# lpylpy0514/VitTracker

Hardware: AMD Instinct MI355X
Metric: track() frames/sec per GPU, vit_48_h32, 128px search / 64px template (higher is better)
Workload: dtype f32

## Files before the change

### vittracker_amd/csrc/vt_head3.h

```cpp
#pragma once
#include "vt_bf3.h"
#include "vt_head.h"

#ifndef VT_F16
#ifndef VT_SEQ3_C2_MAXP
#define VT_SEQ3_C2_MAXP 5
#endif
#ifndef VT_SEQ3_C2_ACT
#define VT_SEQ3_C2_ACT 8
#endif
#ifndef VT_H3_SKIP
#define VT_H3_SKIP 0
#endif
namespace vth3 {

using vth::C;
using vth::W1;
using vth::nchunks;
using vth::ntiles;
using vt3::bf16x8;
using vt3::u32x2;
using vt3::u32x4;
using vt3::split3;
using vt3::join3;
using G = vth::Geo<8>;

constexpr int npairs(int cin) { return (nchunks(cin) + 1) / 2; }
constexpr int img16(int cin, int cout) { return ntiles(cout) * npairs(cin) * 3 * 64; }
constexpr int O3_W1 = 0;
constexpr int O3_W2 = O3_W1 + img16(48, 32);
constexpr int O3_W3 = O3_W2 + img16(32, 16);
constexpr int O3_W4 = O3_W3 + img16(16, 8);
constexpr int TOWER3_STRIDE = O3_W4 + img16(8, 4);

template <int CIN, int COUT, int NW = 4, int ACT = NW, int MAXP_ = 2>
struct HeadConv3 {
    static constexpr int NQ = CIN / 4, NQO = COUT / 4, NCH = nchunks(CIN), NCP = npairs(CIN), NOT = ntiles(COUT);
    static constexpr bool SPLIT_OT = NOT == 2;
    static constexpr int TSTEP = SPLIT_OT ? NW / 2 : ACT;
    static constexpr int NPT = G::NT / TSTEP;
    static_assert(G::NT % TSTEP == 0 && NPT >= 1 && NOT <= 2, "work split");
    static constexpr int MAXP = NCP < MAXP_ ? NCP : MAXP_;
    static constexpr int NPASS = (NCP + MAXP - 1) / MAXP;
    static constexpr int PS_IN = NQ * G::NPIX, PS_OUT = NQO * G::NPIX;
    u32x4 a[2][MAXP][3];

    __device__ __forceinline__ const u32x4* wbase(const u32x4* __restrict__ wimg, int wave) const {
        return wimg + (SPLIT_OT ? (size_t)(wave & 1) * NCP * 192 : 0);
    }
    __device__ __forceinline__ void load_pass(const u32x4* __restrict__ wb, int p0, int n, int lane, u32x4 (&dst)[MAXP][3]) {
#pragma unroll
        for (int k = 0; k < MAXP; ++k)
            if (k < n)
#pragma unroll
                for (int pc = 0; pc < 3; ++pc) dst[k][pc] = wb[((size_t)(p0 + k) * 3 + pc) * 64 + lane];
        __builtin_amdgcn_sched_barrier(0);
    }
    __device__ __forceinline__ void prefetch(const u32x4* __restrict__ wimg, int wave, int lane) {
        load_pass(wbase(wimg, wave), 0, MAXP, lane, a[0]);
    }
    template <bool FIRST = false>
    __device__ __forceinline__ void run(const u32x2* in_map, u32x2* out_map, const u32x4* __restrict__ wimg,
                                        const float* __restrict__ bias, int wave, int lane) {
        if (!SPLIT_OT && wave >= ACT) return;
        if constexpr (FIRST) prefetch(wimg, wave, lane);
        const int q = lane >> 4;
        const int ot = SPLIT_OT ? (wave & 1) : 0, tfirst = SPLIT_OT ? (wave >> 1) : wave;
        f4 acc[NPT];
        const f4 bv = ld4(bias + 16 * ot + 4 * q);
#pragma unroll
        for (int i = 0; i < NPT; ++i) acc[i] = bv;
        const u32x4* __restrict__ wb = wbase(wimg, wave);
        int cb[NPT][3], centre[NPT];
#pragma unroll
        for (int i = 0; i < NPT; ++i) { G::tap_cols(tfirst + TSTEP * i, lane, cb[i]); centre[i] = cb[i][1] + G::P; }
        auto at = [&](int c, int i) {
            int tap, icq;
            if constexpr (NQ % 4 == 0) { const int cc = c < NCH ? c : NCH - 1; tap = (4 * cc) / NQ; icq = 4 * cc - tap * NQ + q; }
            else vtc::decode_quad<NQ>(4 * c + q, tap, icq);
            const int dy = tap / 3, dx = tap - 3 * dy;
            return icq * G::NPIX + dy * G::P + (dx == 0 ? cb[i][0] : (dx == 1 ? cb[i][1] : cb[i][2]));
        };
        auto read_b = [&](int cp, u32x4 (&b)[NPT][3]) {
#pragma unroll
            for (int i = 0; i < NPT; ++i) {
                const int o0 = at(2 * cp, i), o1 = at(2 * cp + 1, i);
#pragma unroll
                for (int pc = 0; pc < 3; ++pc) {
                    const u32x2 lo = in_map[pc * PS_IN + o0], hi = in_map[pc * PS_IN + o1];
                    b[i][pc] = u32x4{lo.x, lo.y, hi.x, hi.y};
                }
            }
        };
        u32x4 b[2][NPT][3];
        read_b(0, b[0]);
#pragma unroll
        for (int p = 0; p < NPASS; ++p) {
            constexpr int LASTN = NCP - (NPASS - 1) * MAXP;
            const int n = p + 1 < NPASS ? MAXP : LASTN;
            if (p + 1 < NPASS) load_pass(wb, (p + 1) * MAXP, p + 2 < NPASS ? MAXP : LASTN, lane, a[(p + 1) & 1]);
#pragma unroll
            for (int k = 0; k < MAXP; ++k) {
                if (k >= n) break;
                const int cp = p * MAXP + k;
                if (cp + 1 < NCP) {
                    read_b(cp + 1, b[(cp + 1) & 1]);
                    __builtin_amdgcn_sched_barrier(0);
                }
                const u32x4 (&w)[3] = a[p & 1][k];
#pragma unroll
                for (int i = 0; i < NPT; ++i) {
                    const u32x4 (&x)[3] = b[cp & 1][i];
                    auto mm = [&](int wp, int xp) {
                        acc[i] = __builtin_amdgcn_mfma_f32_16x16x32_bf16(__builtin_bit_cast(bf16x8, w[wp]), __builtin_bit_cast(bf16x8, x[xp]), acc[i], 0, 0, 0);
                    };
                    mm(2, 0); mm(0, 2); mm(1, 1); mm(1, 0); mm(0, 1); mm(0, 0);
                }
            }
        }
        if (16 * ot + 4 * q < COUT) {
#pragma unroll
            for (int i = 0; i < NPT; ++i) {
                f4 v = acc[i];
                v.x = fmaxf(v.x, 0.f); v.y = fmaxf(v.y, 0.f); v.z = fmaxf(v.z, 0.f); v.w = fmaxf(v.w, 0.f);
                u32x2 h, m, l;
                split3(v, h, m, l);
                const int e = (4 * ot + q) * G::NPIX + centre[i];
                out_map[e] = h; out_map[PS_OUT + e] = m; out_map[2 * PS_OUT + e] = l;
            }
        }
    }
    static constexpr int SP = 3, NSP = (NCP + SP - 1) / SP, SBUF16 = SP * 192;
    static constexpr int pass_n16(int p) { return (p + 1 < NSP ? SP : NCP - (NSP - 1) * SP) * 192; }
    template <typename Pipe>
    __device__ __forceinline__ void run_staged(const u32x2* in_map, u32x2* out_map, const float* __restrict__ bias, int wave, int lane,
                                               int g0, Pipe& pipe) {
        static_assert(NOT == 1 && NPT == 1 && ACT == NW, "staged form: one output tile, one pixel tile per wave");
        const int q = lane >> 4;
        f4 acc = ld4(bias + 4 * q);
        int cb[3];
        G::tap_cols(wave, lane, cb);
        const int centre = cb[1] + G::P;
        auto at = [&](int c) {
            int tap, icq;
            if constexpr (NQ % 4 == 0) { const int cc = c < NCH ? c : NCH - 1; tap = (4 * cc) / NQ; icq = 4 * cc - tap * NQ + q; }
            else vtc::decode_quad<NQ>(4 * c + q, tap, icq);
            const int dy = tap / 3, dx = tap - 3 * dy;
            return icq * G::NPIX + dy * G::P + (dx == 0 ? cb[0] : (dx == 1 ? cb[1] : cb[2]));
        };
        auto read_b = [&](int cp, u32x4 (&b)[3]) {
            const int o0 = at(2 * cp), o1 = at(2 * cp + 1);
#pragma unroll
            for (int pc = 0; pc < 3; ++pc) {
                const u32x2 lo = in_map[pc * PS_IN + o0], hi = in_map[pc * PS_IN + o1];
                b[pc] = u32x4{lo.x, lo.y, hi.x, hi.y};
            }
        };
        u32x4 b[2][3], w[2][3];
        read_b(0, b[0]);
#pragma unroll
        for (int p = 0; p < NSP; ++p) {
            const int n = pass_n16(p) / 192, g = g0 + p;
            pipe.fetch(g + 2);
            const u32x4* sb = pipe.buf(g);
            auto read_w = [&](int k, u32x4 (&ww)[3]) {
#pragma unroll
                for (int pc = 0; pc < 3; ++pc) ww[pc] = sb[(k * 3 + pc) * 64 + lane];
            };
            read_w(0, w[0]);
#pragma unroll
            for (int k = 0; k < SP; ++k) {
                if (k >= n) break;
                const int cp = p * SP + k;
                if (k + 1 < n) read_w(k + 1, w[(k + 1) & 1]);
                if (cp + 1 < NCP) read_b(cp + 1, b[(cp + 1) & 1]);
                __builtin_amdgcn_sched_barrier(0);
                const u32x4 (&x)[3] = b[cp & 1];
                const u32x4 (&ww)[3] = w[k & 1];
                auto mm = [&](int wp, int xp) {
                    acc = __builtin_amdgcn_mfma_f32_16x16x32_bf16(__builtin_bit_cast(bf16x8, ww[wp]), __builtin_bit_cast(bf16x8, x[xp]), acc, 0, 0, 0);
                };
                if (!(VT_H3_SKIP & 2)) { mm(2, 0); mm(0, 2); mm(1, 1); mm(1, 0); mm(0, 1); mm(0, 0); }
            }
            if (p == NSP - 1 && 4 * q < COUT) {
                f4 v = acc;
                v.x = fmaxf(v.x, 0.f); v.y = fmaxf(v.y, 0.f); v.z = fmaxf(v.z, 0.f); v.w = fmaxf(v.w, 0.f);
                u32x2 h, m, l;
                split3(v, h, m, l);
                const int e = q * G::NPIX + centre;
                out_map[e] = h; out_map[PS_OUT + e] = m; out_map[2 * PS_OUT + e] = l;
            }
            pipe.park(g + 1);
            __syncthreads();
        }
    }
};

constexpr int IN_E = 3 * (C / 4) * G::NPIX, M1_E = 3 * (W1 / 4) * G::NPIX, M2_E = 3 * 4 * G::NPIX;
constexpr int TOWERS3_LDS_BYTES = (IN_E + M1_E + M2_E) * 8;
constexpr int SBUF_BYTES = 3 * 192 * 16;
static_assert(IN_E * 8 / 3 >= SBUF_BYTES, "a tower's second staging buffer is its third of the input map (dead after conv1)");
constexpr int FUSED3_LDS_BYTES = (IN_E + 3 * (M1_E + M2_E)) * 8 + 5 * 64 * 4 + 3 * SBUF_BYTES;
static_assert(FUSED3_LDS_BYTES <= 160 * 1024, "LDS");

struct WeightPipe {
    static constexpr int N2 = HeadConv3<W1, 16>::NSP, N3 = HeadConv3<16, 8>::NSP, N4 = HeadConv3<8, 4>::NSP, NP = N2 + N3 + N4;
    const u32x4* tw3;
    u32x4 *buf0, *buf1;
    int tid;
    u32x4 r[2][3];
    static constexpr int off16(int j) {
        return j < N2 ? O3_W2 + j * HeadConv3<W1, 16>::SBUF16 : j < N2 + N3 ? O3_W3 + (j - N2) * HeadConv3<16, 8>::SBUF16 : O3_W4 + (j - N2 - N3) * HeadConv3<8, 4>::SBUF16;
    }
    static constexpr int n16(int j) {
        return j < N2 ? HeadConv3<W1, 16>::pass_n16(j) : j < N2 + N3 ? HeadConv3<16, 8>::pass_n16(j - N2) : HeadConv3<8, 4>::pass_n16(j - N2 - N3);
    }
    __device__ __forceinline__ const u32x4* buf(int j) const { return (j & 1) ? buf1 : buf0; }
    __device__ __forceinline__ void fetch(int j) {
        if (j >= NP) return;
        const u32x4* __restrict__ src = tw3 + off16(j);
#pragma unroll
        for (int k = 0; k < 3; ++k)
            if (tid + 256 * k < n16(j)) r[j & 1][k] = src[tid + 256 * k];
        __builtin_amdgcn_sched_barrier(0);
    }
    __device__ __forceinline__ void park(int j) {
        if (j >= NP) return;
        u32x4* dst = (j & 1) ? buf1 : buf0;
#pragma unroll
        for (int k = 0; k < 3; ++k)
            if (tid + 256 * k < n16(j)) dst[tid + 256 * k] = r[j & 1][k];
    }
};

__device__ __forceinline__ void stage_tokens(u32x2* in_map, const float* __restrict__ feat, int b, int item) {
    const int icq = item >> 6, pix = item & 63;
    u32x2 h, m, l;
    split3(ld4(feat + ((size_t)b * 64 + pix) * C + 4 * icq), h, m, l);
    const int e = icq * G::NPIX + G::interior(pix >> 3, pix & 7);
    in_map[e] = h; in_map[(C / 4) * G::NPIX + e] = m; in_map[2 * (C / 4) * G::NPIX + e] = l;
}

__global__ __launch_bounds__(256) void head_towers3_kernel(const float* __restrict__ feat, const float* __restrict__ hw,
                                                          const u32x4* __restrict__ hw3, float* __restrict__ score,
                                                          float* __restrict__ size, float* __restrict__ offset) {
    extern __shared__ __attribute__((aligned(16))) float sm[];
    u32x2* in_map = reinterpret_cast<u32x2*>(sm);
    u32x2* m1 = in_map + IN_E;
    u32x2* m2 = m1 + M1_E;
    const int b = blockIdx.x, t = blockIdx.y;
    const int lane = threadIdx.x & 63;
    const int wave = __builtin_amdgcn_readfirstlane(threadIdx.x >> 6);
    const float* __restrict__ tw = hw + (size_t)t * vth::TOWER_STRIDE;
    const u32x4* __restrict__ tw3 = hw3 + (size_t)t * TOWER3_STRIDE;
    HeadConv3<C, W1> c1;
    HeadConv3<W1, 16> c2;
    HeadConv3<16, 8> c3;
    HeadConv3<8, 4> c4;
    c1.prefetch(tw3 + O3_W1, wave, lane);
    for (int i = threadIdx.x; i < (IN_E + M1_E + M2_E) / 2; i += 256) reinterpret_cast<u32x4*>(in_map)[i] = u32x4{0, 0, 0, 0};
    __syncthreads();
    for (int i = threadIdx.x; i < 64 * (C / 4); i += 256) stage_tokens(in_map, feat, b, i);
    __syncthreads();
    c2.prefetch(tw3 + O3_W2, wave, lane);
    c1.run(in_map, m1, tw3 + O3_W1, tw + vth::O_B1, wave, lane);
    c3.prefetch(tw3 + O3_W3, wave, lane);
    __syncthreads();
    c2.run(m1, m2, tw3 + O3_W2, tw + vth::O_B2, wave, lane);
    c4.prefetch(tw3 + O3_W4, wave, lane);
    __syncthreads();
    c3.run(m2, m1, tw3 + O3_W3, tw + vth::O_B3, wave, lane);
    __syncthreads();
    c4.run(m1, m2, tw3 + O3_W4, tw + vth::O_B4, wave, lane);
    __syncthreads();
    if (threadIdx.x < 64) {
        const int pix = threadIdx.x, e = G::interior(pix >> 3, pix & 7);
        const f4 v = join3(m2[e], m2[G::NPIX + e], m2[2 * G::NPIX + e]);
        const int nout = (t == 0) ? 1 : 2;
        for (int o = 0; o < nout; ++o) {
            const f4 w5 = ld4(tw + vth::O_W5 + 4 * o);
            float y = tw[vth::O_B5 + o];
            y = fmaf(v.x, w5.x, y); y = fmaf(v.y, w5.y, y); y = fmaf(v.z, w5.z, y); y = fmaf(v.w, w5.w, y);
            if (t == 0) score[(size_t)b * 64 + pix] = sigmoid_clamped(y);
            else if (t == 2) size[((size_t)b * 2 + o) * 64 + pix] = sigmoid_clamped(y);
            else offset[((size_t)b * 2 + o) * 64 + pix] = y;
        }
    }
}

__global__ __launch_bounds__(768) void head_fused3_kernel(const float* __restrict__ feat, const float* __restrict__ hw,
                                                          const u32x4* __restrict__ hw3, const float* __restrict__ window,
                                                          float* __restrict__ score, float* __restrict__ size,
                                                          float* __restrict__ offset, float* __restrict__ pred,
                                                          float* __restrict__ hann, float* __restrict__ conf, TrackTail tail,
                                                          int has_tail) {
    constexpr int F = 8;
    extern __shared__ __attribute__((aligned(16))) float sm[];
    u32x2* in_map = reinterpret_cast<u32x2*>(sm);
    const int b = blockIdx.x;
    const int lane = threadIdx.x & 63;
    const int wave = __builtin_amdgcn_readfirstlane(threadIdx.x >> 6);
    const int t = wave >> 2, wv = wave & 3, tid = threadIdx.x - 256 * t;
    u32x2* m1 = in_map + IN_E + t * (M1_E + M2_E);
    u32x2* m2 = m1 + M1_E;
    float* outs = reinterpret_cast<float*>(in_map + IN_E + 3 * (M1_E + M2_E));
    const float* __restrict__ tw = hw + (size_t)t * vth::TOWER_STRIDE;
    const u32x4* __restrict__ tw3 = hw3 + (size_t)t * TOWER3_STRIDE;
    HeadConv3<C, W1, 4, 4, 1> c1;
    HeadConv3<W1, 16> c2;
    HeadConv3<16, 8> c3;
    HeadConv3<8, 4> c4;
    c1.prefetch(tw3 + O3_W1, wv, lane);
    static_assert(64 * (C / 4) == 768, "one staged element per thread");
    const f4 fv = ld4(feat + ((size_t)b * 64 + (threadIdx.x & 63)) * C + 4 * (threadIdx.x >> 6));
    float win = 0.f;
    if (wave == 0 && window != nullptr) win = window[lane];
    {
        constexpr int NPL = (IN_E + 3 * (M1_E + M2_E)) / G::NPIX, ZU = (G::NPIX - F * G::P) / 2, TOPU = G::P / 2;
        static_assert(G::P % 2 == 0 && G::NPIX % 2 == 0 && ((F + 1) * G::P) % 2 == 0, "16-byte units");
        for (int j = threadIdx.x; j < NPL * ZU; j += 768) {
            const int pl = j / ZU, u = j - pl * ZU;
            reinterpret_cast<u32x4*>(in_map + pl * G::NPIX)[u < TOPU ? u : (F + 1) * G::P / 2 + (u - TOPU)] = u32x4{0, 0, 0, 0};
        }
    }
    {
        const int icq = threadIdx.x >> 6, pix = threadIdx.x & 63;
        u32x2 h, m, l;
        split3(fv, h, m, l);
        const int e = icq * G::NPIX + G::interior(pix >> 3, pix & 7);
        in_map[e] = h; in_map[(C / 4) * G::NPIX + e] = m; in_map[2 * (C / 4) * G::NPIX + e] = l;
    }
    __syncthreads();
    u32x4* const sbuf0 = reinterpret_cast<u32x4*>(outs + 5 * 64) + t * (SBUF_BYTES / 16);
    u32x4* const sbuf1 = reinterpret_cast<u32x4*>(in_map) + t * (IN_E / 6);
    WeightPipe pipe{tw3, sbuf0, sbuf1, tid, {}};
    pipe.fetch(0);
    pipe.fetch(1);
    if (!(VT_H3_SKIP & 1)) c1.run(in_map, m1, tw3 + O3_W1, tw + vth::O_B1, wv, lane);
    pipe.park(0);
    __syncthreads();
    c2.run_staged(m1, m2, tw + vth::O_B2, wv, lane, 0, pipe);
    c3.run_staged(m2, m1, tw + vth::O_B3, wv, lane, WeightPipe::N2, pipe);
    c4.run_staged(m1, m2, tw + vth::O_B4, wv, lane, WeightPipe::N2 + WeightPipe::N3, pipe);
    if (tid < F * F) {
        const int pix = tid, e = G::interior(pix >> 3, pix & 7);
        const f4 v = join3(m2[e], m2[G::NPIX + e], m2[2 * G::NPIX + e]);
        const int nout = (t == 0) ? 1 : 2;
        for (int o = 0; o < nout; ++o) {
            const f4 w5 = ld4(tw + vth::O_W5 + 4 * o);
            float y = tw[vth::O_B5 + o];
            y = fmaf(v.x, w5.x, y); y = fmaf(v.y, w5.y, y); y = fmaf(v.z, w5.z, y); y = fmaf(v.w, w5.w, y);
            if (t == 0) { y = sigmoid_clamped(y); score[(size_t)b * F * F + pix] = y; outs[pix] = y; }
            else if (t == 2) { y = sigmoid_clamped(y); size[((size_t)b * 2 + o) * F * F + pix] = y; outs[(1 + o) * F * F + pix] = y; }
            else { offset[((size_t)b * 2 + o) * F * F + pix] = y; outs[(3 + o) * F * F + pix] = y; }
        }
    }
    __syncthreads();
    if (wave == 0) {
        const float sc = outs[lane];
        float v0 = sc, v1 = window != nullptr ? win * sc : -3.0e38f;
        int i0 = lane, i1 = lane;
#pragma unroll
        for (int off = 32; off > 0; off >>= 1) {
            vth::argmax_merge(v0, i0, __shfl_xor(v0, off, 64), __shfl_xor(i0, off, 64));
            vth::argmax_merge(v1, i1, __shfl_xor(v1, off, 64), __shfl_xor(i1, off, 64));
        }
        if (lane == 0) {
            constexpr int n = F * F;
            const float fF = (float)F;
            const float* sz = outs + n;
            const float* of = outs + 3 * n;
            if (pred != nullptr) {
                pred[b * 4 + 0] = ((float)(i0 % F) + of[i0]) / fF;
                pred[b * 4 + 1] = ((float)(i0 / F) + of[n + i0]) / fF;
                pred[b * 4 + 2] = sz[i0];
                pred[b * 4 + 3] = sz[n + i0];
            }
            if (window != nullptr && (hann != nullptr || has_tail)) {
                const float hb[4] = {((float)(i1 % F) + of[i1]) / fF, ((float)(i1 / F) + of[n + i1]) / fF, sz[i1], sz[n + i1]};
                if (hann != nullptr) {
                    hann[b * 4 + 0] = hb[0];
                    hann[b * 4 + 1] = hb[1];
                    hann[b * 4 + 2] = hb[2];
                    hann[b * 4 + 3] = hb[3];
                }
                if (has_tail) update_state_one(b, hb, v0, tail);
            }
            if (conf != nullptr) conf[b] = v0;
        }
    }
}

using G16 = vth::Geo<16>;
constexpr int SEQ3_IN_E = 3 * (C / 4) * G16::NPIX;
constexpr int SEQ3_LDS_BYTES = SEQ3_IN_E * 8 + (W1 / 4 + 4) * G16::NPIX * 16 + 256 * 4;
static_assert(SEQ3_LDS_BYTES <= 160 * 1024, "LDS");
static_assert((G16::NPIX * 8) % 256 == 128, "piece planes: conflict-free ds_read_b64");

template <int CIN, int COUT, int NW, int MAXP_, int ACT = NW>
struct SeqConvB {
    static constexpr int NQ = CIN / 4, NCH = nchunks(CIN), NCP = npairs(CIN), NOT = ntiles(COUT);
    static constexpr int TSTEP = NOT == 2 ? NW / 2 : ACT, NPT = G16::NT / TSTEP;
    static constexpr int MAXP = NCP < MAXP_ ? NCP : MAXP_;
    static constexpr int NPASS = (NCP + MAXP - 1) / MAXP, LASTN = NCP - (NPASS - 1) * MAXP;
    static constexpr int PS_IN = NQ * G16::NPIX;
    static_assert(NQ % 4 == 0 && G16::NT % TSTEP == 0 && NOT >= 1 && NOT <= 2, "a chunk never straddles two taps; pixel tiles divide over the waves");
    u32x4 a[2][MAXP][3];

    __device__ static __forceinline__ bool active(int wave) { return NOT == 2 || ACT == NW || wave < ACT; }
    __device__ static __forceinline__ int ot_of(int wave) { return NOT == 2 ? (wave & 1) : 0; }
    __device__ static __forceinline__ int tile_of(int wave, int i) { return (NOT == 2 ? (wave >> 1) : wave) + TSTEP * i; }
    __device__ __forceinline__ void load_pass(const u32x4* __restrict__ wb, int p0, int n, int lane, u32x4 (&dst)[MAXP][3]) {
#pragma unroll
        for (int k = 0; k < MAXP; ++k)
            if (k < n)
#pragma unroll
                for (int pc = 0; pc < 3; ++pc) dst[k][pc] = wb[((size_t)(p0 + k) * 3 + pc) * 64 + lane];
        __builtin_amdgcn_sched_barrier(0);
    }
    __device__ __forceinline__ void prefetch(const u32x4* __restrict__ wimg, int wave, int lane) {
        if (active(wave)) load_pass(wimg + (size_t)ot_of(wave) * NCP * 192, 0, MAXP, lane, a[0]);
    }
    __device__ __forceinline__ void compute(const u32x2* in_map, const u32x4* __restrict__ wimg, const float* __restrict__ bias, int wave,
                                            int lane, bool skip, f4 (&acc)[NPT]) {
        const int q = lane >> 4, ot = ot_of(wave);
        const u32x4* __restrict__ wb = wimg + (size_t)ot * NCP * 192;
        const f4 bv = ld4(bias + 16 * ot + 4 * q);
        int base[NPT];
#pragma unroll
// ... 267 lines not shown
```

### vittracker_amd/csrc/vt_weights.h

```cpp
#pragma once

namespace {

using TensorMap = std::map<std::string, std::pair<const float*, int64_t>>;

int need(const TensorMap& tm, const std::string& name, int64_t numel, const float** out) {
    auto it = tm.find(name);
    if (it == tm.end()) return fail(VT_ERR_MISSING_KEY, "missing key in state dict: " + name);
    if (it->second.second != numel)
        return fail(VT_ERR_MISSING_KEY, "shape mismatch for " + name + ": got " + std::to_string(it->second.second) +
                                            " elements, want " + std::to_string(numel));
    *out = it->second.first;
    return VT_OK;
}

int fold_conv_bn(const TensorMap& tm, const std::string& conv, const std::string& bn, bool conv_bias, int cout,
                 int cin, std::vector<double>& w, std::vector<double>& b) {
    const float *pw, *pb = nullptr, *g, *beta, *mu, *var;
    int rc;
    if ((rc = need(tm, conv + ".weight", (int64_t)cout * cin * 9, &pw))) return rc;
    if (conv_bias && (rc = need(tm, conv + ".bias", cout, &pb))) return rc;
    if ((rc = need(tm, bn + ".weight", cout, &g))) return rc;
    if ((rc = need(tm, bn + ".bias", cout, &beta))) return rc;
    if ((rc = need(tm, bn + ".running_mean", cout, &mu))) return rc;
// ... 29 lines not shown
    return out;
}

void pack_conv_quads(const std::vector<double>& w, int cout, int cin, float* dst) {
    const int kp = vth::kpad16(cin);
    for (int g = 0; g < cout / 4; ++g)
        for (int k = 0; k < kp; ++k)
            for (int oc = 0; oc < 4; ++oc)
                dst[((size_t)g * kp + k) * 4 + oc] = k < 9 * cin ? (float)w[((size_t)(4 * g + oc) * cin + k % cin) * 9 + k / cin] : 0.f;
}

void pack_conv_image(const std::vector<double>& w, int cout, int cin, float* dst) {
    const int nq = (cin + 3) / 4, nqt = 9 * nq, nch = (nqt + 3) / 4, not_ = (cout + 15) / 16;
    for (int ot = 0; ot < not_; ++ot)
        for (int c = 0; c < nch; ++c)
            for (int l = 0; l < 64; ++l)
                for (int r = 0; r < 4; ++r) {
                    const int oc = 16 * ot + (l & 15), Q = 4 * c + (l >> 4);
                    float v = 0.f;
                    if (oc < cout && Q < nqt) {
                        const int tap = Q / nq, ic = 4 * (Q % nq) + r;
                        if (ic < cin) v = (float)w[((size_t)oc * cin + ic) * 9 + tap];
                    }
                    dst[(((size_t)ot * nch + c) * 64 + l) * 4 + r] = v;
                }
}

void split3_host(float v, uint16_t (&pieces)[3]) {
    uint32_t xb, r1b, r2b;
    std::memcpy(&xb, &v, 4);
    float hf; const uint32_t hb = xb & 0xffff0000u; std::memcpy(&hf, &hb, 4);
    const float r1 = v - hf; std::memcpy(&r1b, &r1, 4);
    float mf; const uint32_t mb = r1b & 0xffff0000u; std::memcpy(&mf, &mb, 4);
    const float r2 = r1 - mf; std::memcpy(&r2b, &r2, 4);
    pieces[0] = (uint16_t)(xb >> 16); pieces[1] = (uint16_t)(r1b >> 16); pieces[2] = (uint16_t)(r2b >> 16);
}

void pack_k48_image3(const float* img1, int ntiles, uint16_t* dst) {
    constexpr int NC = vtb::NC;
    uint16_t pcs[3];
    for (int ot = 0; ot < ntiles; ++ot) {
        uint16_t* o = dst + (size_t)ot * vtb::W3_FC1_OT16 * 8;
        for (int l = 0; l < 64; ++l) {
            for (int e = 0; e < 8; ++e) {
                split3_host(img1[(((size_t)ot * NC + (e >> 2)) * 64 + l) * 4 + (e & 3)], pcs);
                for (int pc = 0; pc < 3; ++pc) o[((size_t)pc * 64 + l) * 8 + e] = pcs[pc];
            }
            for (int e = 0; e < 4; ++e) {
                split3_host(img1[(((size_t)ot * NC + 2) * 64 + l) * 4 + e], pcs);
                for (int pc = 0; pc < 3; ++pc) o[(size_t)192 * 8 + ((size_t)pc * 64 + l) * 4 + e] = pcs[pc];
            }
        }
    }
}

void pack_mlp_images3(const float* img1, const float* img2, const float* imgqkv, const float* imgproj, uint16_t* dst) {
    constexpr int NC = vtb::NC, NH = vtb::NH;
    uint16_t pcs[3];
    pack_k48_image3(imgqkv, 9, dst + (size_t)(vtb::W3_FC1_TILES + vtb::W3_FC2_TILES) * 512);
    pack_k48_image3(imgproj, NC, dst + (size_t)(vtb::W3_FC1_TILES + vtb::W3_FC2_TILES + vtb::W3_QKV_TILES) * 512);
    for (int ot = 0; ot < NH; ++ot) {
        uint16_t* o = dst + (size_t)ot * vtb::W3_FC1_OT16 * 8;
        for (int l = 0; l < 64; ++l) {
            for (int e = 0; e < 8; ++e) {
                split3_host(img1[(((size_t)ot * NC + (e >> 2)) * 64 + l) * 4 + (e & 3)], pcs);
                for (int pc = 0; pc < 3; ++pc) o[((size_t)pc * 64 + l) * 8 + e] = pcs[pc];
            }
            for (int e = 0; e < 4; ++e) {
                split3_host(img1[(((size_t)ot * NC + 2) * 64 + l) * 4 + e], pcs);
                for (int pc = 0; pc < 3; ++pc) o[(size_t)192 * 8 + ((size_t)pc * 64 + l) * 4 + e] = pcs[pc];
            }
        }
    }
    uint16_t* d2 = dst + (size_t)vtb::W3_FC1_TILES * 512;
    for (int ot = 0; ot < NC; ++ot)
        for (int p = 0; p < NH / 2; ++p)
            for (int l = 0; l < 64; ++l)
                for (int e = 0; e < 8; ++e) {
                    split3_host(img2[(((size_t)ot * NH + 2 * p + (e >> 2)) * 64 + l) * 4 + (e & 3)], pcs);
                    for (int pc = 0; pc < 3; ++pc) d2[((((size_t)ot * (NH / 2) + p) * 3 + pc) * 64 + l) * 8 + e] = pcs[pc];
                }
}

void pack_conv_image3(const std::vector<double>& w, int cout, int cin, uint16_t* dst) {
    const int nq = (cin + 3) / 4, nqt = 9 * nq, nch = (nqt + 3) / 4, ncp = (nch + 1) / 2, not_ = (cout + 15) / 16;
    for (int ot = 0; ot < not_; ++ot)
        for (int cp = 0; cp < ncp; ++cp)
            for (int l = 0; l < 64; ++l)
                for (int e = 0; e < 8; ++e) {
                    const int c = 2 * cp + (e >> 2), r = e & 3;
                    const int oc = 16 * ot + (l & 15), Q = 4 * c + (l >> 4);
                    float v = 0.f;
                    if (oc < cout && c < nch && Q < nqt) {
                        const int tap = Q / nq, ic = 4 * (Q % nq) + r;
                        if (ic < cin) v = (float)w[((size_t)oc * cin + ic) * 9 + tap];
                    }
                    uint16_t pieces[3];
                    split3_host(v, pieces);
                    for (int pc = 0; pc < 3; ++pc) dst[((((size_t)ot * ncp + cp) * 3 + pc) * 64 + l) * 8 + e] = pieces[pc];
                }
}

void pack_linear_image(const float* W, int OUT, int IN, float* dst) {
    const int nc = IN / 16;
    for (int ot = 0; ot < OUT / 16; ++ot)
        for (int c = 0; c < nc; ++c)
            for (int l = 0; l < 64; ++l)
                for (int r = 0; r < 4; ++r)
                    dst[(((size_t)ot * nc + c) * 64 + l) * 4 + r] = W[(size_t)(16 * ot + (l & 15)) * IN + 16 * c + 4 * (l >> 4) + r];
}

int upload(DevBuf& d, const std::vector<float>& h) {
    if (!d.p || d.n != h.size()) {
        d.release();
        int rc = d.alloc(h.size());
        if (rc) return rc;
    }
    HIP_TRY(hipMemcpy(d.p, h.data(), h.size() * sizeof(float), hipMemcpyHostToDevice));
    return VT_OK;
}

std::vector<float> hann2d(int F) {
    std::vector<float> w1(F), w((size_t)F * F);
    const float k = (float)(2.0 * M_PI / (F + 1));
    for (int i = 0; i < F; ++i) w1[i] = 0.5f * (1.0f - cosf(k * (float)(i + 1)));
    for (int y = 0; y < F; ++y)
        for (int x = 0; x < F; ++x) w[(size_t)y * F + x] = w1[y] * w1[x];
    return w;
}

int fold_w1u(vt_model* m, const float* mean3, const float* std3) {
    const std::vector<double>& w = m->stem_w1_f64;
    const std::vector<double>& b = m->stem_b1_f64;
    if (w.size() != 6 * 3 * 9 || b.size() != 6) return fail(VT_ERR_STATE, "layer-1 weights not loaded");
    std::vector<double> wf(w.size());
    std::vector<float> img(vts::W1U_FLOATS, 0.f);
    for (int j = 0; j < 6; ++j) {
        double bias = b[j];
        for (int c = 0; c < 3; ++c)
            for (int t = 0; t < 9; ++t) {
                const double wv = w[((size_t)j * 3 + c) * 9 + t];
                wf[((size_t)j * 3 + c) * 9 + t] = wv / (255.0 * (double)std3[c]);
                bias += wv * (-(double)mean3[c] / (double)std3[c]);
            }
        img[vts::W1U_BIAS + j] = (float)bias;
    }
    const std::vector<float> sec = pack_conv_sections(wf, 6, 3);
    std::copy(sec.begin(), sec.end(), img.begin());
    for (int c = 0; c < 3; ++c) img[vts::W1U_PAD + c] = (float)(255.0 * (double)mean3[c]);
    if (int rc = upload(m->stem_w1u, img)) return rc;
    for (int c = 0; c < 3; ++c) {
        m->norm_mean[c] = mean3[c];
        m->norm_std[c] = std3[c];
    }
    return VT_OK;
}

int load_weights_generic(vt_model* m, const TensorMap& tm) {
    const vtg::Dims d = m->gd;
    const int C = d.C, HID = d.hid();
    int rc;
    const int sch[5] = {3, C / 8, C / 4, C / 2, C};
    for (int i = 0; i < 4; ++i) {
        const std::string p = "patch_embed.net." + std::to_string(2 * i);
        std::vector<double> w, b;
        if ((rc = fold_conv_bn(tm, p + ".c", p + ".bn", false, sch[i + 1], sch[i], w, b))) return rc;
        if ((rc = upload(m->g_stem_w[i], std::vector<float>(w.begin(), w.end())))) return rc;
        if ((rc = upload(m->g_stem_b[i], std::vector<float>(b.begin(), b.end())))) return rc;
    }
    const float* p;
    if ((rc = need(tm, "pos_embed_z", (int64_t)m->len_z * C, &p))) return rc;
    if ((rc = upload(m->pos_z, std::vector<float>(p, p + (size_t)m->len_z * C)))) return rc;
    if ((rc = need(tm, "pos_embed_x", (int64_t)m->len_x * C, &p))) return rc;
    if ((rc = upload(m->pos_x, std::vector<float>(p, p + (size_t)m->len_x * C)))) return rc;
// ... 116 lines not shown
    std::vector<float> bp((size_t)m->cfg.depth * vtb::BLOCK_STRIDE + 2 * C);
    std::vector<uint16_t> bp3((size_t)m->cfg.depth * vtb::BLOCK3_STRIDE * 2, 0);
    for (int b = 0; b < m->cfg.depth; ++b) {
        const std::string pre = "blocks." + std::to_string(b) + ".";
        float* dst = bp.data() + (size_t)b * vtb::BLOCK_STRIDE;
        struct V { const char* name; int off; int n; };
        const V vecs[] = {{"norm1.weight", vtb::O_LN1G, C}, {"norm1.bias", vtb::O_LN1B, C},
                          {"attn.qkv.bias", vtb::O_BQKV, 3 * C}, {"attn.proj.bias", vtb::O_BPROJ, C},
                          {"norm2.weight", vtb::O_LN2G, C}, {"norm2.bias", vtb::O_LN2B, C},
                          {"mlp.fc1.bias", vtb::O_B1, 4 * C}, {"mlp.fc2.bias", vtb::O_B2, C}};
        for (const V& v : vecs) {
            if ((rc = need(tm, pre + v.name, v.n, &p))) return rc;
            std::memcpy(dst + v.off, p, v.n * sizeof(float));
        }
        auto fold_ln = [&](const char* wname, int out, int o_ln_g, int o_ln_b, int o_bias, int o_w) -> int {
            const float* W;
            int rc2 = need(tm, pre + wname, (int64_t)out * C, &W);
            if (rc2) return rc2;
            std::vector<float> wf((size_t)out * C);
            for (int o = 0; o < out; ++o) {
                double acc = (double)dst[o_bias + o];
                for (int i = 0; i < C; ++i) {
                    wf[(size_t)o * C + i] = (float)((double)W[(size_t)o * C + i] * (double)dst[o_ln_g + i]);
                    acc += (double)W[(size_t)o * C + i] * (double)dst[o_ln_b + i];
                }
                dst[o_bias + o] = (float)acc;
            }
            pack_linear_image(wf.data(), out, C, dst + o_w);
            return VT_OK;
        };
        if ((rc = fold_ln("attn.qkv.weight", 3 * C, vtb::O_LN1G, vtb::O_LN1B, vtb::O_BQKV, vtb::O_WQKV))) return rc;
        if ((rc = need(tm, pre + "attn.proj.weight", C * C, &p))) return rc;
        pack_linear_image(p, C, C, dst + vtb::O_WPROJ);
        if ((rc = fold_ln("mlp.fc1.weight", 4 * C, vtb::O_LN2G, vtb::O_LN2B, vtb::O_B1, vtb::O_W1))) return rc;
        if ((rc = need(tm, pre + "mlp.fc2.weight", 4 * C * C, &p))) return rc;
        pack_linear_image(p, C, 4 * C, dst + vtb::O_W2);
        pack_mlp_images3(dst + vtb::O_W1, dst + vtb::O_W2, dst + vtb::O_WQKV, dst + vtb::O_WPROJ, bp3.data() + (size_t)b * vtb::BLOCK3_STRIDE * 2);
    }
    {
        float* dst = bp.data() + (size_t)m->cfg.depth * vtb::BLOCK_STRIDE;
        if ((rc = need(tm, "norm.weight", C, &p))) return rc;
        std::memcpy(dst, p, C * sizeof(float));
        if ((rc = need(tm, "norm.bias", C, &p))) return rc;
        std::memcpy(dst + C, p, C * sizeof(float));
    }
    if ((rc = upload(m->blocks, bp))) return rc;
#ifdef VT_F16
    {
        const size_t nflt = (size_t)m->cfg.depth * vtb::BLOCK_STRIDE;
        m->blocks3.release();
        if ((rc = m->blocks3.alloc(nflt / 2 + 256 + 256))) return rc;
        hipLaunchKernelGGL(f32_to_opnd_kernel, dim3((unsigned)((nflt / 4 + 255) / 256)), dim3(256), 0, nullptr, m->blocks.p,
                           reinterpret_cast<_Float16*>(m->blocks3.p), nflt / 4);
        HIP_TRY(hipGetLastError());
        HIP_TRY(hipDeviceSynchronize());
    }
#else
    {
        std::vector<float> as_f(bp3.size() / 2);
        std::memcpy(as_f.data(), bp3.data(), bp3.size() * 2);
        if ((rc = upload(m->blocks3, as_f))) return rc;
    }
#endif
    std::vector<float> hp((size_t)3 * vth::TOWER_STRIDE, 0.f);
#ifndef VT_F16
    std::vector<uint16_t> hp3((size_t)3 * vth3::TOWER3_STRIDE * 8, 0);
#endif
    const char* towers[3] = {"ctr", "offset", "size"};
    const int chans[5] = {48, 32, 16, 8, 4};
    const int woff[4] = {vth::O_W1, vth::O_W2, vth::O_W3, vth::O_W4};
    const int boff[4] = {vth::O_B1, vth::O_B2, vth::O_B3, vth::O_B4};
    for (int t = 0; t < 3; ++t) {
        float* dst = hp.data() + (size_t)t * vth::TOWER_STRIDE;
        for (int i = 0; i < 4; ++i) {
            const std::string cn = std::string("box_head.conv") + std::to_string(i + 1) + "_" + towers[t];
            std::vector<double> w, b;
            if ((rc = fold_conv_bn(tm, cn + ".0", cn + ".1", true, chans[i + 1], chans[i], w, b))) return rc;
            pack_conv_image(w, chans[i + 1], chans[i], dst + woff[i]);
            if (i == 2) pack_conv_quads(w, 8, 16, dst + vth::O_W3Q);
            if (i == 3) pack_conv_quads(w, 4, 8, dst + vth::O_W4Q);
#ifndef VT_F16
            {
                const int woff3[4] = {vth3::O3_W1, vth3::O3_W2, vth3::O3_W3, vth3::O3_W4};
                pack_conv_image3(w, chans[i + 1], chans[i], hp3.data() + ((size_t)t * vth3::TOWER3_STRIDE + woff3[i]) * 8);
            }
#endif
            for (int o = 0; o < chans[i + 1]; ++o) dst[boff[i] + o] = (float)b[o];
        }
        const int nout = t == 0 ? 1 : 2;
        const std::string c5 = std::string("box_head.conv5_") + towers[t];
        if ((rc = need(tm, c5 + ".weight", nout * 4, &p))) return rc;
        std::memcpy(dst + vth::O_W5, p, nout * 4 * sizeof(float));
        if ((rc = need(tm, c5 + ".bias", nout, &p))) return rc;
        std::memcpy(dst + vth::O_B5, p, nout * sizeof(float));
    }
    if ((rc = upload(m->head, hp))) return rc;
#ifdef VT_F16
    for (int t = 0; t < 3; ++t)
        for (int i = 0; i < 4; ++i) {
            const int sizes[4] = {vth::O_B1 - vth::O_W1, vth::O_B2 - vth::O_W2, vth::O_B3 - vth::O_W3, vth::O_B4 - vth::O_W4};
            if ((rc = opnd_inplace(m->head.p + (size_t)t * vth::TOWER_STRIDE + woff[i], (size_t)sizes[i]))) return rc;
        }
#endif
#ifndef VT_F16
    {
        std::vector<float> as_f(hp3.size() / 2);
        std::memcpy(as_f.data(), hp3.data(), hp3.size() * 2);
        if ((rc = upload(m->head3, as_f))) return rc;
    }
#endif
    m->weights_loaded = true;
    return VT_OK;
}

}
```

Baseline: 3.375 million.

## Store head conv activation maps as channel octets for single 16-byte LDS reads

Changes the LDS activation map layout of the split-bf16 head convolutions from 4-channel quads (8-byte elements) to 8-channel octets (16-byte elements). Each B-operand fetch becomes one 16-byte LDS read per piece instead of two 8-byte reads joined together. The weight packing is reordered to match the octet K ordering, and padded octets in the last pair are clamped one pair back. Output stores and input staging now write 8-byte halves into the octet layout. The address selection per lane adds some ALU work, and the weight packing path depends on m->F==8.

```diff
diff --git a/vittracker_amd/csrc/vt_head3.h b/vittracker_amd/csrc/vt_head3.h
--- a/vittracker_amd/csrc/vt_head3.h
+++ b/vittracker_amd/csrc/vt_head3.h
@@ -35,15 +35,35 @@
 
 template <int CIN, int COUT, int NW = 4, int ACT = NW, int MAXP_ = 2>
 struct HeadConv3 {
-    static constexpr int NQ = CIN / 4, NQO = COUT / 4, NCH = nchunks(CIN), NCP = npairs(CIN), NOT = ntiles(COUT);
+    static constexpr int NO = CIN / 8, NOO = (COUT + 7) / 8, NOCT = 9 * NO, NCP = npairs(CIN), NOT = ntiles(COUT);
+    static_assert(CIN % 8 == 0 && 4 * NCP >= NOCT && 4 * NCP - NOCT < 4 && NOCT >= 4, "whole octets; the last pair's pad octets clamp one pair back");
     static constexpr bool SPLIT_OT = NOT == 2;
     static constexpr int TSTEP = SPLIT_OT ? NW / 2 : ACT;
     static constexpr int NPT = G::NT / TSTEP;
     static_assert(G::NT % TSTEP == 0 && NPT >= 1 && NOT <= 2, "work split");
     static constexpr int MAXP = NCP < MAXP_ ? NCP : MAXP_;
     static constexpr int NPASS = (NCP + MAXP - 1) / MAXP;
-    static constexpr int PS_IN = NQ * G::NPIX, PS_OUT = NQO * G::NPIX;
+    static constexpr int PS_IN = NO * G::NPIX, PS_OUT = NOO * G::NPIX;
     u32x4 a[2][MAXP][3];
+
+    __device__ static __forceinline__ int at(int cp, int q, int qoff, const int (&cb)[3]) {
+        auto cand = [&](int j) {
+            int o = 4 * cp + j;
+            if (o >= NOCT) o -= 4;
+            const int tap = o / NO, oct = o - tap * NO, dy = tap / 3, dx = tap - 3 * dy;
+            return (oct - j) * G::NPIX + dy * G::P + (dx == 0 ? cb[0] : (dx == 1 ? cb[1] : cb[2]));
+        };
+        const int c0 = cand(0), c1 = cand(1), c2 = cand(2), c3 = cand(3);
+        return qoff + (q < 2 ? (q < 1 ? c0 : c1) : (q < 3 ? c2 : c3));
+    }
+    __device__ static __forceinline__ int out_half(int ot, int q, int pix) { return 2 * (((4 * ot + q) >> 1) * G::NPIX + pix) + (q & 1); }
+    __device__ static __forceinline__ void store3(u32x4* out_map, int e, f4 v) {
+        v.x = fmaxf(v.x, 0.f); v.y = fmaxf(v.y, 0.f); v.z = fmaxf(v.z, 0.f); v.w = fmaxf(v.w, 0.f);
+        u32x2 h, m, l;
+        split3(v, h, m, l);
+        u32x2* o2 = reinterpret_cast<u32x2*>(out_map);
+        o2[e] = h; o2[2 * PS_OUT + e] = m; o2[4 * PS_OUT + e] = l;
+    }
 
     __device__ __forceinline__ const u32x4* wbase(const u32x4* __restrict__ wimg, int wave) const {
         return wimg + (SPLIT_OT ? (size_t)(wave & 1) * NCP * 192 : 0);
@@ -60,11 +80,11 @@
         load_pass(wbase(wimg, wave), 0, MAXP, lane, a[0]);
     }
     template <bool FIRST = false>
-    __device__ __forceinline__ void run(const u32x2* in_map, u32x2* out_map, const u32x4* __restrict__ wimg,
+    __device__ __forceinline__ void run(const u32x4* in_map, u32x4* out_map, const u32x4* __restrict__ wimg,
                                         const float* __restrict__ bias, int wave, int lane) {
         if (!SPLIT_OT && wave >= ACT) return;
         if constexpr (FIRST) prefetch(wimg, wave, lane);
-        const int q = lane >> 4;
+        const int q = lane >> 4, qoff = q * G::NPIX;
         const int ot = SPLIT_OT ? (wave & 1) : 0, tfirst = SPLIT_OT ? (wave >> 1) : wave;
         f4 acc[NPT];
         const f4 bv = ld4(bias + 16 * ot + 4 * q);
@@ -74,22 +94,12 @@
         int cb[NPT][3], centre[NPT];
 #pragma unroll
         for (int i = 0; i < NPT; ++i) { G::tap_cols(tfirst + TSTEP * i, lane, cb[i]); centre[i] = cb[i][1] + G::P; }
-        auto at = [&](int c, int i) {
-            int tap, icq;
-            if constexpr (NQ % 4 == 0) { const int cc = c < NCH ? c : NCH - 1; tap = (4 * cc) / NQ; icq = 4 * cc - tap * NQ + q; }
-            else vtc::decode_quad<NQ>(4 * c + q, tap, icq);
-            const int dy = tap / 3, dx = tap - 3 * dy;
-            return icq * G::NPIX + dy * G::P + (dx == 0 ? cb[i][0] : (dx == 1 ? cb[i][1] : cb[i][2]));
-        };
         auto read_b = [&](int cp, u32x4 (&b)[NPT][3]) {
 #pragma unroll
             for (int i = 0; i < NPT; ++i) {
-                const int o0 = at(2 * cp, i), o1 = at(2 * cp + 1, i);
-#pragma unroll
-                for (int pc = 0; pc < 3; ++pc) {
-                    const u32x2 lo = in_map[pc * PS_IN + o0], hi = in_map[pc * PS_IN + o1];
-                    b[i][pc] = u32x4{lo.x, lo.y, hi.x, hi.y};
-                }
+                const int o = at(cp, q, qoff, cb[i]);
+#pragma unroll
+                for (int pc = 0; pc < 3; ++pc) b[i][pc] = in_map[pc * PS_IN + o];
             }
         };
         u32x4 b[2][NPT][3];
@@ -120,41 +130,24 @@
         }
         if (16 * ot + 4 * q < COUT) {
 #pragma unroll
-            for (int i = 0; i < NPT; ++i) {
-                f4 v = acc[i];
-                v.x = fmaxf(v.x, 0.f); v.y = fmaxf(v.y, 0.f); v.z = fmaxf(v.z, 0.f); v.w = fmaxf(v.w, 0.f);
-                u32x2 h, m, l;
-                split3(v, h, m, l);
-                const int e = (4 * ot + q) * G::NPIX + centre[i];
-                out_map[e] = h; out_map[PS_OUT + e] = m; out_map[2 * PS_OUT + e] = l;
-            }
+            for (int i = 0; i < NPT; ++i) store3(out_map, out_half(ot, q, centre[i]), acc[i]);
         }
     }
     static constexpr int SP = 3, NSP = (NCP + SP - 1) / SP, SBUF16 = SP * 192;
     static constexpr int pass_n16(int p) { return (p + 1 < NSP ? SP : NCP - (NSP - 1) * SP) * 192; }
     template <typename Pipe>
-    __device__ __forceinline__ void run_staged(const u32x2* in_map, u32x2* out_map, const float* __restrict__ bias, int wave, int lane,
+    __device__ __forceinline__ void run_staged(const u32x4* in_map, u32x4* out_map, const float* __restrict__ bias, int wave, int lane,
                                                int g0, Pipe& pipe) {
         static_assert(NOT == 1 && NPT == 1 && ACT == NW, "staged form: one output tile, one pixel tile per wave");
-        const int q = lane >> 4;
+        const int q = lane >> 4, qoff = q * G::NPIX;
         f4 acc = ld4(bias + 4 * q);
         int cb[3];
         G::tap_cols(wave, lane, cb);
         const int centre = cb[1] + G::P;
-        auto at = [&](int c) {
-            int tap, icq;
-            if constexpr (NQ % 4 == 0) { const int cc = c < NCH ? c : NCH - 1; tap = (4 * cc) / NQ; icq = 4 * cc - tap * NQ + q; }
-            else vtc::decode_quad<NQ>(4 * c + q, tap, icq);
-            const int dy = tap / 3, dx = tap - 3 * dy;
-            return icq * G::NPIX + dy * G::P + (dx == 0 ? cb[0] : (dx == 1 ? cb[1] : cb[2]));
-        };
         auto read_b = [&](int cp, u32x4 (&b)[3]) {
-            const int o0 = at(2 * cp), o1 = at(2 * cp + 1);
-#pragma unroll
-            for (int pc = 0; pc < 3; ++pc) {
-                const u32x2 lo = in_map[pc * PS_IN + o0], hi = in_map[pc * PS_IN + o1];
-                b[pc] = u32x4{lo.x, lo.y, hi.x, hi.y};
-            }
+            const int o = at(cp, q, qoff, cb);
+#pragma unroll
+            for (int pc = 0; pc < 3; ++pc) b[pc] = in_map[pc * PS_IN + o];
         };
         u32x4 b[2][3], w[2][3];
         read_b(0, b[0]);
@@ -182,25 +175,18 @@
                 };
                 if (!(VT_H3_SKIP & 2)) { mm(2, 0); mm(0, 2); mm(1, 1); mm(1, 0); mm(0, 1); mm(0, 0); }
             }
-            if (p == NSP - 1 && 4 * q < COUT) {
-                f4 v = acc;
-                v.x = fmaxf(v.x, 0.f); v.y = fmaxf(v.y, 0.f); v.z = fmaxf(v.z, 0.f); v.w = fmaxf(v.w, 0.f);
-                u32x2 h, m, l;
-                split3(v, h, m, l);
-                const int e = q * G::NPIX + centre;
-                out_map[e] = h; out_map[PS_OUT + e] = m; out_map[2 * PS_OUT + e] = l;
-            }
+            if (p == NSP - 1 && 4 * q < COUT) store3(out_map, out_half(0, q, centre), acc);
             pipe.park(g + 1);
             __syncthreads();
         }
     }
 };
 
-constexpr int IN_E = 3 * (C / 4) * G::NPIX, M1_E = 3 * (W1 / 4) * G::NPIX, M2_E = 3 * 4 * G::NPIX;
-constexpr int TOWERS3_LDS_BYTES = (IN_E + M1_E + M2_E) * 8;
+constexpr int IN_E = 3 * (C / 8) * G::NPIX, M1_E = 3 * (W1 / 8) * G::NPIX, M2_E = 3 * 2 * G::NPIX;
+constexpr int TOWERS3_LDS_BYTES = (IN_E + M1_E + M2_E) * 16;
 constexpr int SBUF_BYTES = 3 * 192 * 16;
-static_assert(IN_E * 8 / 3 >= SBUF_BYTES, "a tower's second staging buffer is its third of the input map (dead after conv1)");
-constexpr int FUSED3_LDS_BYTES = (IN_E + 3 * (M1_E + M2_E)) * 8 + 5 * 64 * 4 + 3 * SBUF_BYTES;
+static_assert(IN_E * 16 / 3 >= SBUF_BYTES, "a tower's second staging buffer is its third of the input map (dead after conv1)");
+constexpr int FUSED3_LDS_BYTES = (IN_E + 3 * (M1_E + M2_E)) * 16 + 5 * 64 * 4 + 3 * SBUF_BYTES;
 static_assert(FUSED3_LDS_BYTES <= 160 * 1024, "LDS");
 
 struct WeightPipe {
@@ -233,21 +219,29 @@
     }
 };
 
-__device__ __forceinline__ void stage_tokens(u32x2* in_map, const float* __restrict__ feat, int b, int item) {
+__device__ __forceinline__ void stage_quad(u32x4* in_map, f4 v, int icq, int pix) {
+    u32x2 h, m, l;
+    split3(v, h, m, l);
+    u32x2* im2 = reinterpret_cast<u32x2*>(in_map);
+    const int e = 2 * ((icq >> 1) * G::NPIX + G::interior(pix >> 3, pix & 7)) + (icq & 1);
+    im2[e] = h; im2[2 * (C / 8) * G::NPIX + e] = m; im2[4 * (C / 8) * G::NPIX + e] = l;
+}
+__device__ __forceinline__ void stage_tokens(u32x4* in_map, const float* __restrict__ feat, int b, int item) {
     const int icq = item >> 6, pix = item & 63;
-    u32x2 h, m, l;
-    split3(ld4(feat + ((size_t)b * 64 + pix) * C + 4 * icq), h, m, l);
-    const int e = icq * G::NPIX + G::interior(pix >> 3, pix & 7);
-    in_map[e] = h; in_map[(C / 4) * G::NPIX + e] = m; in_map[2 * (C / 4) * G::NPIX + e] = l;
+    stage_quad(in_map, ld4(feat + ((size_t)b * 64 + pix) * C + 4 * icq), icq, pix);
+}
+__device__ __forceinline__ f4 join_low(const u32x4* m2, int e) {
+    const u32x2* h2 = reinterpret_cast<const u32x2*>(m2);
+    return join3(h2[2 * e], h2[2 * (G::NPIX + e)], h2[2 * (2 * G::NPIX + e)]);
 }
 
 __global__ __launch_bounds__(256) void head_towers3_kernel(const float* __restrict__ feat, const float* __restrict__ hw,
                                                           const u32x4* __restrict__ hw3, float* __restrict__ score,
                                                           float* __restrict__ size, float* __restrict__ offset) {
     extern __shared__ __attribute__((aligned(16))) float sm[];
-    u32x2* in_map = reinterpret_cast<u32x2*>(sm);
-    u32x2* m1 = in_map + IN_E;
-    u32x2* m2 = m1 + M1_E;
+    u32x4* in_map = reinterpret_cast<u32x4*>(sm);
+    u32x4* m1 = in_map + IN_E;
+    u32x4* m2 = m1 + M1_E;
     const int b = blockIdx.x, t = blockIdx.y;
     const int lane = threadIdx.x & 63;
     const int wave = __builtin_amdgcn_readfirstlane(threadIdx.x >> 6);
@@ -258,7 +252,7 @@
     HeadConv3<16, 8> c3;
     HeadConv3<8, 4> c4;
     c1.prefetch(tw3 + O3_W1, wave, lane);
-    for (int i = threadIdx.x; i < (IN_E + M1_E + M2_E) / 2; i += 256) reinterpret_cast<u32x4*>(in_map)[i] = u32x4{0, 0, 0, 0};
+    for (int i = threadIdx.x; i < IN_E + M1_E + M2_E; i += 256) in_map[i] = u32x4{0, 0, 0, 0};
     __syncthreads();
     for (int i = threadIdx.x; i < 64 * (C / 4); i += 256) stage_tokens(in_map, feat, b, i);
     __syncthreads();
@@ -275,7 +269,7 @@
     __syncthreads();
     if (threadIdx.x < 64) {
         const int pix = threadIdx.x, e = G::interior(pix >> 3, pix & 7);
-        const f4 v = join3(m2[e], m2[G::NPIX + e], m2[2 * G::NPIX + e]);
+        const f4 v = join_low(m2, e);
         const int nout = (t == 0) ? 1 : 2;
         for (int o = 0; o < nout; ++o) {
             const f4 w5 = ld4(tw + vth::O_W5 + 4 * o);
@@ -296,13 +290,13 @@
                                                           int has_tail) {
     constexpr int F = 8;
     extern __shared__ __attribute__((aligned(16))) float sm[];
-    u32x2* in_map = reinterpret_cast<u32x2*>(sm);
+    u32x4* in_map = reinterpret_cast<u32x4*>(sm);
     const int b = blockIdx.x;
     const int lane = threadIdx.x & 63;
     const int wave = __builtin_amdgcn_readfirstlane(threadIdx.x >> 6);
     const int t = wave >> 2, wv = wave & 3, tid = threadIdx.x - 256 * t;
-    u32x2* m1 = in_map + IN_E + t * (M1_E + M2_E);
-    u32x2* m2 = m1 + M1_E;
+    u32x4* m1 = in_map + IN_E + t * (M1_E + M2_E);
+    u32x4* m2 = m1 + M1_E;
     float* outs = reinterpret_cast<float*>(in_map + IN_E + 3 * (M1_E + M2_E));
     const float* __restrict__ tw = hw + (size_t)t * vth::TOWER_STRIDE;
     const u32x4* __restrict__ tw3 = hw3 + (size_t)t * TOWER3_STRIDE;
@@ -316,23 +310,16 @@
     float win = 0.f;
     if (wave == 0 && window != nullptr) win = window[lane];
     {
-        constexpr int NPL = (IN_E + 3 * (M1_E + M2_E)) / G::NPIX, ZU = (G::NPIX - F * G::P) / 2, TOPU = G::P / 2;
-        static_assert(G::P % 2 == 0 && G::NPIX % 2 == 0 && ((F + 1) * G::P) % 2 == 0, "16-byte units");
+        constexpr int NPL = (IN_E + 3 * (M1_E + M2_E)) / G::NPIX, ZU = G::NPIX - F * G::P, TOPU = G::P;
         for (int j = threadIdx.x; j < NPL * ZU; j += 768) {
             const int pl = j / ZU, u = j - pl * ZU;
-            reinterpret_cast<u32x4*>(in_map + pl * G::NPIX)[u < TOPU ? u : (F + 1) * G::P / 2 + (u - TOPU)] = u32x4{0, 0, 0, 0};
-        }
-    }
-    {
-        const int icq = threadIdx.x >> 6, pix = threadIdx.x & 63;
-        u32x2 h, m, l;
-        split3(fv, h, m, l);
-        const int e = icq * G::NPIX + G::interior(pix >> 3, pix & 7);
-        in_map[e] = h; in_map[(C / 4) * G::NPIX + e] = m; in_map[2 * (C / 4) * G::NPIX + e] = l;
-    }
+            in_map[pl * G::NPIX + (u < TOPU ? u : (F + 1) * G::P + (u - TOPU))] = u32x4{0, 0, 0, 0};
+        }
+    }
+    stage_quad(in_map, fv, threadIdx.x >> 6, threadIdx.x & 63);
     __syncthreads();
     u32x4* const sbuf0 = reinterpret_cast<u32x4*>(outs + 5 * 64) + t * (SBUF_BYTES / 16);
-    u32x4* const sbuf1 = reinterpret_cast<u32x4*>(in_map) + t * (IN_E / 6);
+    u32x4* const sbuf1 = in_map + t * (IN_E / 3);
     WeightPipe pipe{tw3, sbuf0, sbuf1, tid, {}};
     pipe.fetch(0);
     pipe.fetch(1);
@@ -344,7 +331,7 @@
     c4.run_staged(m1, m2, tw + vth::O_B4, wv, lane, WeightPipe::N2 + WeightPipe::N3, pipe);
     if (tid < F * F) {
         const int pix = tid, e = G::interior(pix >> 3, pix & 7);
-        const f4 v = join3(m2[e], m2[G::NPIX + e], m2[2 * G::NPIX + e]);
+        const f4 v = join_low(m2, e);
         const int nout = (t == 0) ? 1 : 2;
         for (int o = 0; o < nout; ++o) {
             const f4 w5 = ld4(tw + vth::O_W5 + 4 * o);
diff --git a/vittracker_amd/csrc/vt_weights.h b/vittracker_amd/csrc/vt_weights.h
--- a/vittracker_amd/csrc/vt_weights.h
+++ b/vittracker_amd/csrc/vt_weights.h
@@ -135,14 +135,14 @@
                 }
 }
 
-void pack_conv_image3(const std::vector<double>& w, int cout, int cin, uint16_t* dst) {
+void pack_conv_image3(const std::vector<double>& w, int cout, int cin, uint16_t* dst, bool octets = false) {
     const int nq = (cin + 3) / 4, nqt = 9 * nq, nch = (nqt + 3) / 4, ncp = (nch + 1) / 2, not_ = (cout + 15) / 16;
     for (int ot = 0; ot < not_; ++ot)
         for (int cp = 0; cp < ncp; ++cp)
             for (int l = 0; l < 64; ++l)
                 for (int e = 0; e < 8; ++e) {
-                    const int c = 2 * cp + (e >> 2), r = e & 3;
-                    const int oc = 16 * ot + (l & 15), Q = 4 * c + (l >> 4);
+                    const int r = e & 3, oc = 16 * ot + (l & 15);
+                    const int Q = octets ? 2 * (4 * cp + (l >> 4)) + (e >> 2) : 4 * (2 * cp + (e >> 2)) + (l >> 4), c = Q / 4;
                     float v = 0.f;
                     if (oc < cout && c < nch && Q < nqt) {
                         const int tap = Q / nq, ic = 4 * (Q % nq) + r;
@@ -425,7 +425,7 @@
 #ifndef VT_F16
             {
                 const int woff3[4] = {vth3::O3_W1, vth3::O3_W2, vth3::O3_W3, vth3::O3_W4};
-                pack_conv_image3(w, chans[i + 1], chans[i], hp3.data() + ((size_t)t * vth3::TOWER3_STRIDE + woff3[i]) * 8);
+                pack_conv_image3(w, chans[i + 1], chans[i], hp3.data() + ((size_t)t * vth3::TOWER3_STRIDE + woff3[i]) * 8, m->F == 8);
             }
 #endif
             for (int o = 0; o < chans[i + 1]; ++o) dst[boff[i] + o] = (float)b[o];
```

Result: no change. 3.395 million (median of 6 runs) (+0.6%).
